# hdm0922/PathTracerDemo

Measured on AMD Instinct MI355X. Metric: Msamples/sec at 1920x1080, 1 spp ReSTIR DI; per-pixel L2 vs WebGPU ref, higher is better.
Workload: dtype f32; 1 GPU; c3_interior_32 reuse 1920x1080, 1 spp/frame (configs[2]); frame=1920x1080, band_rows_per_gpu=1080, parallelism=row-bands x1

## Files before the change

### pathtracerdemo_amd/csrc/ptx_reuse.hip

```cpp
#include "ptx_wave_common.h"

namespace ptx {

constexpr uint32_t SALT_TEMPORAL = 0x54454D50u, SALT_SPATIAL = 0x53504154u;

enum : uint32_t { JS_HDR, JS_F, JS_CUR, JS_NRM, JS_PREV, JS_RRF, JS_COUNT };
constexpr uint32_t kJobFresh = 1u << 24;
constexpr uint32_t kResReuseLayout = 0x100u;
#ifndef PTX_JOB_FRESH
#define PTX_JOB_FRESH 1
#endif

struct Job {
    uint32_t i, length, phase, seed1, idx, matref;
    uint32_t k, lab;
    bool shift, rok;
    int32_t ref;
    int32_t dom;
    f3 f;
    float prod;
    Surface cur;
    f3 prev;
    float beta, rr_p;
    f3 rr_f;
};

__device__ __forceinline__ uint32_t job_id(const ReuseArgs &A, uint32_t pix, uint32_t slot) {
    return pix * A.jpx + slot * A.jslot;
}
__device__ __forceinline__ const uint4 *res_at(const uint4 *base, int32_t idx) { return base + 8 * (ptrdiff_t)idx; }
constexpr int32_t kHistRef = 1 << 30;
__device__ __forceinline__ const uint4 *res_of(const ReuseArgs &A, int32_t ref) {
    return ref >= (kHistRef >> 1) ? A.hist + 8 * (ptrdiff_t)(ref - kHistRef) : A.cur + 8 * (ptrdiff_t)ref;
}
constexpr int32_t kDomPrev = INT32_MIN;

__device__ __forceinline__ uint32_t job_hw(const Job &s) {
    return s.i | (s.length << 8) | (s.phase << 16) | (s.lab << 18) | (s.rok ? 1u << 21 : 0u) |
           (s.shift ? 1u << 22 : 0u) | (s.k << 25);
}
__device__ __forceinline__ void job_unhw(Job &s, uint32_t hw) {
    s.i = hw & 0xffu; s.length = (hw >> 8) & 0xffu; s.phase = (hw >> 16) & 3u;
    s.lab = (hw >> 18) & 7u; s.rok = (hw >> 21) & 1u; s.shift = (hw >> 22) & 1u; s.k = (hw >> 25) & 7u;
}
__device__ __forceinline__ void job_store(const ReuseArgs &A, uint32_t jid, const Job &s) {
    const size_t n = A.njobs;
    float4 *st = A.jstate;
    if (PTX_JOB_FRESH && s.i == 1u && s.phase == 0u && s.dom != kDomPrev) {
        st[JS_HDR * n + jid] = make_float4(asf(job_hw(s) | kJobFresh), asf((uint32_t)s.dom), asf(s.idx),
                                           asf((uint32_t)s.ref));
        st[JS_F * n + jid] = make_float4(s.rr_f.x, s.rr_f.y, s.rr_f.z, s.prod);
        st[JS_RRF * n + jid] = make_float4(s.beta, s.rr_p, 0.0f, 0.0f);
        return;
    }
    st[JS_HDR * n + jid] = make_float4(asf(job_hw(s)), asf(s.seed1), asf(s.idx), asf((uint32_t)s.ref));
    st[JS_F * n + jid] = make_float4(s.f.x, s.f.y, s.f.z, s.prod);
    if (s.phase == 1u) return;
    st[JS_CUR * n + jid] = make_float4(s.cur.pos.x, s.cur.pos.y, s.cur.pos.z, asf(s.matref));
    st[JS_NRM * n + jid] = make_float4(s.cur.nrm.x, s.cur.nrm.y, s.cur.nrm.z, s.beta);
    st[JS_PREV * n + jid] = make_float4(s.prev.x, s.prev.y, s.prev.z, s.rr_p);
    st[JS_RRF * n + jid] = make_float4(s.rr_f.x, s.rr_f.y, s.rr_f.z, 0.0f);
}
__device__ __forceinline__ void job_load(const Scene &sc, const ReuseArgs &A, uint32_t jid, Job &s) {
    const size_t n = A.njobs;
    const float4 *st = A.jstate;
    const float4 hd = st[JS_HDR * n + jid], fv = st[JS_F * n + jid];
    const uint32_t hw = asu(hd.x);
    job_unhw(s, hw);
    s.idx = asu(hd.z); s.ref = (int32_t)asu(hd.w);
    s.prod = fv.w;
    const bool fresh = (hw & kJobFresh) != 0u;
    uint32_t seed1 = asu(hd.y), matref = 0u;
    int32_t dom = s.dom;
    f3 f = mk(fv.x, fv.y, fv.z), rr_f = mk(0.0f, 0.0f, 0.0f), prev = rr_f;
    float beta = 0.0f, rr_p = 0.0f;
    Surface cur{};
    if (fresh) {
        const float4 rf = st[JS_RRF * n + jid];
        dom = (int32_t)asu(hd.y);
        seed1 = res_of(A, s.ref)[0].y;
        f = mk(1.0f, 1.0f, 1.0f);
        rr_f = mk(fv.x, fv.y, fv.z);
        beta = rf.x; rr_p = rf.y;
        (void)surf_load(sc, A.surf, dom, cur, matref);
        const int32_t W = (int32_t)sc.width, q = dom >= 0 ? dom / W : -((-dom + W - 1) / W);
        prev = x0_of(sc, (uint32_t)(dom - q * W), (uint32_t)((int32_t)sc.row_begin + q));
    } else if (s.phase != 1u) {
        const float4 cu = st[JS_CUR * n + jid], nr = st[JS_NRM * n + jid];
        const float4 pv = st[JS_PREV * n + jid], rf = st[JS_RRF * n + jid];
        matref = asu(cu.w);
        cur.pos = mk(cu.x, cu.y, cu.z);
        cur.nrm = mk(nr.x, nr.y, nr.z);
        cur.mat = material_at(sc, matref);
        beta = nr.w;
        prev = mk(pv.x, pv.y, pv.z); rr_p = pv.w;
        rr_f = mk(rf.x, rf.y, rf.z);
    }
    s.seed1 = seed1; s.matref = matref; s.dom = dom;
    s.f = f; s.rr_f = rr_f; s.prev = prev;
    s.beta = beta; s.rr_p = rr_p;
    s.cur = cur;
}

__device__ __forceinline__ bool rr_step(Job &s, const Surface &X, f3 L, f3 fv, float pdf) {
    s.rr_f = s.rr_f * (fv * fabsf(dot(X.nrm, L)));
    s.rr_p *= pdf;
    const float ps = luminance(s.rr_f) / s.rr_p;
    const bool ok = ps > 0.0f;
    s.rr_p *= ps;
    if (ps > 1.0f) s.beta /= ps;
    return ok;
}

__device__ __forceinline__ void job_init(Job &s, f3 x0, const Surface &X1, uint32_t matref, int32_t ref,
                                         uint32_t length, uint32_t seed1, int32_t dom, uint32_t k, bool shift) {
    s.i = 1u; s.length = length; s.phase = 0u; s.seed1 = seed1; s.idx = 0u; s.ref = ref; s.dom = dom;
    s.k = min(k, 7u); s.lab = 0u; s.shift = shift; s.rok = false;
    s.f = mk(1.0f, 1.0f, 1.0f); s.prod = 1.0f;
    s.prev = x0;
    s.cur = X1;
    s.matref = matref;
    s.beta = 1.0f; s.rr_p = 1.0f; s.rr_f = mk(1.0f, 1.0f, 1.0f);
}
__device__ __forceinline__ bool job_begin(const Scene &sc, const ReuseArgs &A, Job &s, uint32_t x, uint32_t y,
                                          int32_t dom, int32_t ref) {
    const uint4 *rv = res_at(A.cur, ref);
    const uint4 r5 = rv[5];
    const uint32_t C = rv[7].y, length = r5.w;
    Surface X1;
    uint32_t matref;
    if (C == 0u || length < 2u || !surf_load(sc, A.surf, dom, X1, matref)) return false;
    job_init(s, x0_of(sc, x, y), X1, matref, ref, length, rv[0].y, dom, r5.x & 0xffu, false);
    return true;
}
__device__ __forceinline__ bool job_hyb(const Job &s) { return s.k >= 2u && s.k < s.length; }
__device__ __forceinline__ bool rough_under(const Surface &X, uint32_t lobe) {
    return (lobe == LOBE_LAMBERT ? 1.0f : X.mat.rough) >= RECONNECTION_ROUGHNESS;
}
__device__ __forceinline__ bool safe_edge(bool ra, bool rb, f3 a, f3 b) {
    return length(a - b) >= RECONNECTION_DISTANCE && ra && rb;
}
__device__ __forceinline__ float rc_geo(f3 prev, const Surface &Xk) {
    const f3 dv = Xk.pos - prev;
    const float d2 = dot(dv, dv);
    const float ck = fabsf(dot(Xk.nrm, dv / __builtin_sqrtf(d2)));
    return d2 / ck;
}
__device__ __forceinline__ uint4 rc_next(const uint4 *rv, uint32_t w20) {
    return (w20 & kResReuseLayout) ? rv[0] : rv[6];
}

enum : int { JK_ANY = -1, JK_L = 0, JK_C = 1, JK_B = 2 };
__device__ __forceinline__ int job_kind(uint32_t length, uint32_t k) {
    return length <= 2u ? JK_L : (k == 2u ? JK_C : JK_B);
}
template <int KIND = JK_ANY>
__device__ __forceinline__ bool job_emit(const Scene &sc, const Seg &g, const ReuseArgs &A, bool emit, Job &s,
                                         uint32_t jid, uint32_t seed0) {
    bool ray = false, vis = false, go = false;
    f3 o = mk(0.0f, 0.0f, 0.0f), d = o, Le = o;
    float remain = -1.0f;
    if (emit) {
        const uint4 *rv = res_of(A, s.ref);
        const f3 V = normalize(s.prev - s.cur.pos);
        const bool hyb = job_hyb(s);
        bool ok = true;
        if (KIND == JK_ANY ? s.i + 1u < s.length : KIND != JK_L) {
            const bool conn = KIND == JK_ANY ? s.shift && hyb && s.i + 1u == s.k : KIND == JK_C;
            const bool fixd = KIND == JK_ANY && s.shift && hyb && s.i == s.k;
            f3 dir;
            uint32_t lobe = LOBE_LAMBERT;
            if (conn || fixd) {
                const uint4 r5 = rv[5];
                const Surface Xt = get_surface(sc, gdecode(conn ? rv[4] : rc_next(rv, r5.x)));
                if (conn) {
                    const bool rk1 = rough_under(s.cur, r5.y), rk = rough_under(Xt, r5.z);
                    if (s.i >= 2u && s.lab == 0u && safe_edge(s.rok, rk1, s.prev, s.cur.pos)) s.lab = s.i;
                    if (s.lab == 0u && safe_edge(rk1, rk, s.cur.pos, Xt.pos)) s.lab = s.k;
                    ok = s.lab == s.k;
                }
                const f3 dv = Xt.pos - s.cur.pos;
                dir = dv / length(dv);
            } else {
                uint32_t seed = s.i == 1u ? seed0 : s.seed1;
                dir = sample_bsdf(seed, s.cur, V, lobe);
            }
            float pdf;
            const f3 fv = bsdf_pdf(s.cur, V, dir, pdf);
            if (!conn && !fixd && (!hyb || s.i + 2u <= s.k)) s.prod *= pdf;
            ok = rr_step(s, s.cur, dir, fv, pdf) && ok;
            if (s.shift && !conn && !fixd) {
                const bool rl = rough_under(s.cur, lobe);
                if (s.i >= 2u && s.lab == 0u && safe_edge(s.rok, rl, s.prev, s.cur.pos)) s.lab = s.i;
                s.rok = rl;
            }
            s.phase = conn ? 2u : (fixd ? 3u : 0u);
            o = s.cur.pos; d = dir;
            ray = ok && !fixd;
            go = ok;
        } else {
            const LightSample XL = load_xl(rv);
            if (s.shift && !hyb) {
                const uint32_t ll = XL.type == LIGHT_ENV ? (s.k == s.length ? rv[5].y : LOBE_GGX) : LOBE_LAMBERT;
                const bool rl = rough_under(s.cur, ll);
                if (s.i >= 2u && s.lab == 0u && safe_edge(s.rok, rl, s.prev, s.cur.pos)) s.lab = s.i;
                if (s.lab == 0u) {
                    const bool rough = s.cur.mat.rough >= RECONNECTION_ROUGHNESS;
                    const bool dirl = XL.type == LIGHT_DIRECTION || XL.type == LIGHT_ENV;
                    if ((dirl || length(s.cur.pos - XL.pos) >= RECONNECTION_DISTANCE) && rough) s.lab = s.length;
                }
                ok = s.lab == s.k;
            }
            const f3 L = direction_to_light(s.cur, XL);
            if (XL.type == LIGHT_ENV) {
                float pdf;
                const f3 fv = bsdf_pdf(s.cur, V, L, pdf);
                ok = rr_step(s, s.cur, L, fv, pdf) && ok;
            }
            s.f = s.f * (bsdf(s.cur, L, V) * fabsf(dot(s.cur.nrm, L)));
            float gl = 1.0f;
            if (XL.type == LIGHT_RECT) {
                const f3 r = XL.pos - s.cur.pos;
                const f3 Ld = normalize(r);
                gl = fabsf(dot(get_light(sc, (uint32_t)XL.id).dir, Ld)) / dot(r, r);
            }
            s.prod = hyb ? s.prod / s.beta : s.prod / (gl * s.beta);
            Le = l_emit<true>(XL, s.cur);
            s.phase = 1u;
            const float dist = length(XL.pos - s.cur.pos);
            o = s.cur.pos; d = (XL.pos - s.cur.pos) / dist; remain = dist;
            vis = true;
            ray = go = ok;
        }
        if (!go) A.jres[jid] = make_float4(0.0f, 0.0f, 0.0f, 0.0f);
    }
    const uint32_t idx = g.rbase + wave_alloc(g.l_ray, ray ? 1u : 0u);
    if (ray) {
        s.idx = idx;
        put_ray(g.rays, idx, o, d, remain, vis ? Q_VIS : Q_CLOSEST);
        if (vis) g.res_out[2u * idx] = make_float4(0.0f, Le.x, Le.y, Le.z);
    }
    return go;
}

__device__ __forceinline__ void job_finish(const Seg &g, const JobLists &JL, const ReuseArgs &A, bool live,
                                           const Job &s, uint32_t jid) {
    if (live) job_store(A, jid, s);
    const bool fold = live && A.fold_last && s.phase == 1u;
    if (fold) A.jres[jid] = make_float4(asf(s.idx), asf(g.out_sel), 0.0f, asf(kJobPending));
    job_keep(g, JL, live && !fold, live && s.phase == 1u, jid);
}

#ifndef JOB_STEP_WAVES
#define JOB_STEP_WAVES 4
#endif
__device__ __forceinline__ uint32_t job_step_segment(const Scene &sc, const WaveBufs &w, uint32_t round,
                                                     const ReuseArgs &A, uint32_t *lds) {
    const JobLists JL = job_lists(w, lds);
    const Seg g = seg_begin(w, round, lds);
    uint32_t nh;
    const uint32_t n = split_count(g, nh);
    for (uint32_t base = 0; base < n; base += WB) {
        const uint32_t q = base + threadIdx.x;
        bool emit = false;
        uint32_t jid = 0u;
        Job s;
        if (q < n) {
            jid = split_at(g, JL, q, nh);
            job_load(sc, A, jid, s);
            if (s.phase != 1u) {
                bool ok = true;
                Surface next;
                uint32_t nref = 0u;
                if (s.phase == 0u) {
                    const Hit h = get_hit(g.res_in, s.idx);
                    ok = h.valid;
                    if (ok) {
                        next = surface_at(sc, h.s, h.pos);
                        nref = mat_index(sc, h.s.inst, h.s.mat);
                    }
                } else {
                    const uint4 *rv = res_of(A, s.ref);
                    const Compact cc = gdecode(s.phase == 2u ? rv[4] : rc_next(rv, rv[5].x));
                    next = get_surface(sc, cc);
                    nref = mat_index(sc, cc.inst, cc.mat);
                    if (s.phase == 2u) {
                        const Hit h = get_hit(g.res_in, s.idx);
                        ok = !(h.valid && h.t < length(next.pos - s.cur.pos) * 0.999f);
                    }
                }
                if (!ok) {
                    A.jres[jid] = make_float4(0.0f, 0.0f, 0.0f, 0.0f);
                } else {
                    const f3 V = normalize(s.prev - s.cur.pos);
                    const f3 L = normalize(next.pos - s.cur.pos);
                    s.f = s.f * (bsdf(s.cur, L, V) * fabsf(dot(s.cur.nrm, L)));
                    if (s.phase == 2u || (!s.shift && job_hyb(s) && s.i + 1u == s.k))
                        s.prod = s.prod * rc_geo(s.cur.pos, next);
                    s.prev = s.cur.pos;
                    s.cur = next;
                    s.matref = nref;
                    s.i += 1u;
                    emit = true;
                }
            } else {
                const float4 a = g.res_in[2u * s.idx];
                s.f = s.f * (mk(a.y, a.z, a.w) * a.x);
                const float qv = s.prod;
                const bool valid = qv > 0.0f && qv <= 3.402823466e38f;
                A.jres[jid] = valid ? make_float4(s.f.x, s.f.y, s.f.z, qv) : make_float4(0.0f, 0.0f, 0.0f, 0.0f);
            }
        }
        const bool live = job_emit(sc, g, A, emit, s, jid, 0u);
        job_finish(g, JL, A, live, s, jid);
    }
    job_seg_end(w, g, JL);
    return *g.l_ray;
}
__global__ __launch_bounds__(WB) __attribute__((amdgpu_waves_per_eu(JOB_STEP_WAVES, 8)))
void wjob_step(Scene sc, WaveBufs w, uint32_t round, ReuseArgs A) {
    PTX_WAVE_TIMER(sc, KID_JOB_STEP | (w.seg_base ? 0x80u : 0u));
    __shared__ uint32_t lds[3];
    (void)job_step_segment(sc, w, round, A, lds);
}

__device__ __forceinline__ uint32_t reuse_seed(const Scene &sc, uint32_t x, uint32_t y, uint32_t salt) {
    return pcg(pcg(x * 1973u + y * 9277u + sc.U[U_FRAME] * 26699u) ^ salt);
}
__device__ __forceinline__ bool wrs_update(float &w_sum, float wt, uint32_t &seed) {
    w_sum += wt;
    return rnd(seed) < wt / w_sum;
}
struct SelF { bool known; f3 f; };
__device__ __forceinline__ SelF job_f(float4 r) { return SelF{r.w > 0.0f, mk(r.x, r.y, r.z)}; }
__device__ __forceinline__ float4 job_result(const ReuseArgs &A, const WaveBufs &w, float4 r, uint32_t jid) {
    if (asu(r.w) != kJobPending || asu(r.x) >= A.ray_cap || asu(r.y) >= w.nres) return r;
    const float4 a = w.res[asu(r.y)][2u * asu(r.x)], fv = A.jstate[JS_F * (size_t)A.njobs + jid];
    const f3 f = mk(fv.x, fv.y, fv.z) * (mk(a.y, a.z, a.w) * a.x);
    const float qv = fv.w;
    const bool valid = qv > 0.0f && qv <= 3.402823466e38f;
    return valid ? make_float4(f.x, f.y, f.z, qv) : make_float4(0.0f, 0.0f, 0.0f, 0.0f);
}
__device__ __forceinline__ float4 job_at(const ReuseArgs &A, const WaveBufs &w, uint32_t pix, uint32_t slot) {
    const uint32_t jid = job_id(A, pix, slot);
    return job_result(A, w, A.jres[jid], jid);
}
__device__ __forceinline__ SelF stored_f(const uint4 *r) {
    const uint4 r6 = r[6], r7 = r[7];
    return SelF{r7.w == 1u, mk(asf(r6.z), asf(r6.w), asf(r7.z))};
}
__device__ __forceinline__ void write_reused(uint4 *out, const uint4 *src, float p_sel, float q_sel, SelF fs,
                                             float w_sum, uint32_t C) {
    uint4 a0 = src[0], a5 = src[5];
    const uint4 a1 = src[1], a2 = src[2], a3 = src[3], a4 = src[4];
    if (fs.known && !(a5.x & kResReuseLayout)) {
        const uint32_t k = a5.x & 0xffu;
        if (k >= 2u && k + 1u < a5.w) a0 = src[6];
        a5.x |= kResReuseLayout;
    }
    out[0] = a0; out[1] = a1; out[2] = a2; out[3] = a3; out[4] = a4; out[5] = a5;
    out[6] = make_uint4(asu(p_sel), asu(q_sel), fs.known ? asu(fs.f.x) : 0u, fs.known ? asu(fs.f.y) : 0u);
    out[7] = make_uint4(asu(p_sel > 0.0f ? w_sum / p_sel : 0.0f), C, fs.known ? asu(fs.f.z) : 0u, fs.known ? 1u : 0u);
}

constexpr uint32_t kNbrEscape = 0xFFFFFFFFu;
__device__ __forceinline__ uint4 nbr_pack(bool valid, uint4 r5, uint4 r6, uint4 r7) {
    uint32_t w = 0u;
    const uint32_t k = r5.x & 0xffu;
    if (valid)
        w = (r5.w > 0xfu || k > 0xfu || r7.y > 0x7ffffeu) ? kNbrEscape : (1u << 31) | (r5.w << 27) | (k << 23) | r7.y;
    return make_uint4(r6.x, r6.y, r7.x, w);
}

__device__ __forceinline__ bool temporal_from_init(const Scene &sc, const WaveBufs &w, const ReuseArgs &A, Job &s,
                                                   uint32_t pix, uint32_t jid) {
    const uint4 *rv = res_at(A.cur, s.ref);
    const bool hyb = job_hyb(s);
    while (s.i + 1u < s.length) {
        f3 V = normalize(s.prev - s.cur.pos);
        uint32_t seed = s.i == 1u ? rv[0].x : s.seed1, lobe;
        const f3 dir = sample_bsdf(seed, s.cur, V, lobe);
        float pdf;
        const f3 fv = bsdf_pdf(s.cur, V, dir, pdf);
        if (!hyb || s.i + 2u <= s.k) s.prod *= pdf;
        if (!rr_step(s, s.cur, dir, fv, pdf)) {
            A.jres[jid] = make_float4(0.0f, 0.0f, 0.0f, 0.0f);
            return false;
        }
        const float4 c = w.state[(s.i == 1u ? kStateCs2 : kStateCs3) * w.npix + pix];
        const Surface next = get_surface(sc, gdecode(make_uint4(asu(c.x), asu(c.y), asu(c.z), asu(c.w))));
        V = normalize(s.prev - s.cur.pos);
        const f3 L = normalize(next.pos - s.cur.pos);
        s.f = s.f * (bsdf(s.cur, L, V) * fabsf(dot(s.cur.nrm, L)));
        if (hyb && s.i + 1u == s.k) s.prod = s.prod * rc_geo(s.cur.pos, next);
        s.prev = s.cur.pos;
        s.cur = next;
        s.i += 1u;
    }
    const float T = w.state[kStateTsel * w.npix + pix].x;
    if (T < 0.0f) return true;
    const LightSample XL = load_xl(rv);
    const f3 V = normalize(s.prev - s.cur.pos);
    const f3 L = direction_to_light(s.cur, XL);
    s.f = s.f * (bsdf(s.cur, L, V) * fabsf(dot(s.cur.nrm, L)));
    float gl = 1.0f;
    if (XL.type == LIGHT_RECT) {
        const f3 r = XL.pos - s.cur.pos;
        const f3 Ld = normalize(r);
        gl = fabsf(dot(get_light(sc, (uint32_t)XL.id).dir, Ld)) / dot(r, r);
    }
    s.prod = hyb ? s.prod / s.beta : s.prod / (gl * s.beta);
    const f3 Le = l_emit<true>(XL, s.cur);
    s.f = s.f * (Le * T);
    const float qv = s.prod;
    const bool valid = qv > 0.0f && qv <= 3.402823466e38f;
    A.jres[jid] = valid ? make_float4(s.f.x, s.f.y, s.f.z, qv) : make_float4(0.0f, 0.0f, 0.0f, 0.0f);
    return false;
}

__global__ __launch_bounds__(WB) __attribute__((amdgpu_waves_per_eu(2, 8)))
void wtemporal_start(Scene sc, WaveBufs w, ReuseArgs A) {
    PTX_WAVE_TIMER(sc, KID_TEMP_START | (w.seg_base ? 0x80u : 0u));
    __shared__ uint32_t lds[3];
    const JobLists JL = job_lists(w, lds);
    const Seg g = seg_begin(w, 0u, lds);
    const uint32_t np = padded_pixels(sc);
    for (uint32_t k = 0; k < w.seg_px; k += WB) {
        const uint32_t q = seg_pixel(w, g.j, k);
        uint32_t x, y, pix = 0u;
        bool active = false;
        Job s;
        if (q < np && tile_xy(sc, q, x, y)) {
            pix = (y - sc.row_begin) * sc.width + x;
            active = job_begin(sc, A, s, x, y, (int32_t)pix, (int32_t)pix);
            if (active && A.use_init) active = temporal_from_init(sc, w, A, s, pix, pix);
        }
        const bool live = job_emit(sc, g, A, active, s, pix, active ? A.cur[8u * (size_t)pix].x : 0u);
        job_finish(g, JL, A, live, s, pix);
    }
    job_seg_end(w, g, JL);
}

__global__ __launch_bounds__(WB) void wtemporal_combine(Scene sc, WaveBufs w, ReuseArgs A) {
    PTX_WAVE_TIMER(sc, KID_TEMP_COMBINE | (w.seg_base ? 0x80u : 0u));
    const uint32_t j = w.seg_base + blockIdx.x, np = padded_pixels(sc);
    for (uint32_t k = 0; k < w.seg_px; k += WB) {
        const uint32_t q = seg_pixel(w, j, k);
        uint32_t x, y;
        if (q >= np || !tile_xy(sc, q, x, y)) continue;
        const uint32_t pix = (y - sc.row_begin) * sc.width + x;
        if (!gdecode(A.gbuf[pix]).valid) {
            A.nbr_out[pix] = make_uint4(0u, 0u, 0u, 0u);
            continue;
        }
        uint4 *rv = A.cur + 8u * (size_t)pix;
        const uint4 *hv = A.hist + 8u * (size_t)pix;
        uint32_t seed = reuse_seed(sc, x, y, SALT_TEMPORAL);
        const uint4 r5 = rv[5], r7 = rv[7];
        const float4 er = (r7.y != 0u && r5.w >= 2u) ? job_result(A, w, A.jres[pix], pix) : make_float4(0.0f, 0.0f, 0.0f, 0.0f);
        const float2 ec = make_float2(er.w > 0.0f ? luminance(mk(er.x, er.y, er.z)) : 0.0f, er.w);
        const bool canon_ok = ec.y > 0.0f && ec.x > 0.0f;
        const uint4 h5 = hv[5], h6 = hv[6], h7 = hv[7];
        const uint32_t Cp = A.hist_valid ? min(h7.y, A.cap) : 0u;
        const float cp = (float)Cp, tot = 1.0f + cp;
// ... 632 lines not shown
```

### pathtracerdemo_amd/csrc/ptx_shading.h

```cpp
#pragma once

#include "ptx_device.h"

namespace ptx {

struct Material { f3 albedo; float metal, rough, trans, ior; };
struct Surface { f3 pos, nrm; Material mat; };

__device__ __forceinline__ uint32_t mat_index(const Scene &sc, uint32_t inst, uint32_t sub) {
    return sc.insts[inst].sub_base + sub;
}
__device__ __forceinline__ Material material_at(const Scene &sc, uint32_t flat) {
    const float4 a = sc.mats[2u * flat], b = sc.mats[2u * flat + 1u];
    Material m;
    m.albedo = mk(a.x, a.y, a.z);
    m.metal = a.w;
    m.rough = b.x;
    m.trans = b.y;
    m.ior = b.z;
    return m;
}
__device__ __forceinline__ float get_transmission(const Scene &sc, uint32_t inst, uint32_t mid) {
    return sc.mats[2u * mat_index(sc, inst, mid) + 1u].y;
}
__device__ __forceinline__ float subs_transmission(const SubRoot *subs, const Inst *insts, uint32_t inst, uint32_t mid) {
    return asf(subs[insts[inst].sub_base + mid].pad);
}

__device__ __forceinline__ Surface get_surface(const Scene &sc, Compact x) {
    const Inst &I = sc.insts[x.inst];
    Surface s;
    s.mat = material_at(sc, I.sub_base + x.mat);
    const TriVerts tv = tri_verts(sc, I.tri_base + x.prim);
    f3 p0 = inst_point(I, I.m, tv.p[0]);
    f3 n0 = inst_point_t(I, I.minv, tv.n[0]);
    f3 p1 = inst_point(I, I.m, tv.p[1]);
    f3 n1 = inst_point_t(I, I.minv, tv.n[1]);
    f3 p2 = inst_point(I, I.m, tv.p[2]);
    f3 n2 = inst_point_t(I, I.minv, tv.n[2]);
    float U = x.bu, V = x.bv, W = 1.0f - U - V;
    s.nrm = normalize((n0 * U + n1 * V) + n2 * W);
    s.pos = (p0 * U + p1 * V) + p2 * W;
    return s;
}
__device__ __forceinline__ Surface surface_at(const Scene &sc, const Compact &x, f3 pos) {
    const Inst &I = sc.insts[x.inst];
    Surface s;
    s.mat = material_at(sc, I.sub_base + x.mat);
    const TriVerts tv = tri_verts(sc, I.tri_base + x.prim);
    f3 n0 = inst_point_t(I, I.minv, tv.n[0]);
    f3 n1 = inst_point_t(I, I.minv, tv.n[1]);
    f3 n2 = inst_point_t(I, I.minv, tv.n[2]);
    float U = x.bu, V = x.bv, W = 1.0f - U - V;
    s.nrm = normalize((n0 * U + n1 * V) + n2 * W);
    s.pos = pos;
    return s;
}
__device__ __forceinline__ f3 get_surface_pos(const Scene &sc, Compact x) {
    const Inst &I = sc.insts[x.inst];
    const TriVerts tv = tri_verts(sc, I.tri_base + x.prim);
    f3 p0 = inst_point(I, I.m, tv.p[0]);
    f3 p1 = inst_point(I, I.m, tv.p[1]);
    f3 p2 = inst_point(I, I.m, tv.p[2]);
    float U = x.bu, V = x.bv, W = 1.0f - U - V;
    return (p0 * U + p1 * V) + p2 * W;
}

struct Light { f3 pos, dir, color, U, V; uint32_t type; float intensity, area; };
struct LightSample { f3 dir; uint32_t type; f3 pos; int32_t id; f3 Le; float pdf; };

__device__ __forceinline__ Light get_light(const Scene &sc, uint32_t id) {
    const uint32_t *p = sc.S + sc.U[U_OFF_LIGHT] + STRIDE_LIGHT * id;
    Light l;
    l.pos = mk(asf(p[0]), asf(p[1]), asf(p[2]));
    l.dir = mk(asf(p[3]), asf(p[4]), asf(p[5]));
    l.color = mk(asf(p[6]), asf(p[7]), asf(p[8]));
    l.U = mk(asf(p[9]), asf(p[10]), asf(p[11]));
    l.V = mk(asf(p[12]), asf(p[13]), asf(p[14]));
    l.type = p[15];
    l.intensity = asf(p[16]);
    l.area = asf(p[17]);
    return l;
}
__device__ __forceinline__ float light_cdf(const Scene &sc, uint32_t i) { return asf(sc.S[sc.U[U_OFF_CDF] + i]); }

__device__ __forceinline__ float ggx_d(float NdotH, float R) {
    float a = R * R, a2 = a * a;
    float X = NdotH * NdotH * (a2 - 1.0f) + 1.0f;
    float denom = PI_F * X * X;
    return a2 / fmaxf(denom, EPS_F);
}
__device__ __forceinline__ float geom_shadow(float NdotV, float NdotL, float R) {
    float r = R + 1.0f;
    float K = r * r / 8.0f;
    return 1.0f / ((NdotV * (1.0f - K) + K) * (NdotL * (1.0f - K) + K));
}
__device__ __forceinline__ float pow5(float x) {
    float x2 = x * x;
    return (x2 * x2) * x;
}
__device__ __forceinline__ void fsincos(float x, float &s, float &c) {
    int j = (int)(x * 1.27323954473516f);
    float y = (float)j;
    if (j & 1) {
        j += 1;
        y += 1.0f;
    }
    j &= 7;
    float z = ((x - y * 0.78515625f) - y * 2.4187564849853515625e-4f) - y * 3.77489497744594108e-8f;
    float zz = z * z;
    float ps = ((-1.9515295891e-4f * zz + 8.3321608736e-3f) * zz - 1.6666654611e-1f) * zz * z + z;
    float pc = ((2.443315711809948e-5f * zz - 1.388731625493765e-3f) * zz + 4.166664568298827e-2f) * zz * zz -
               0.5f * zz + 1.0f;
    const bool swap = (j & 2) != 0;
    const float sv = swap ? pc : ps, cv = swap ? ps : pc;
    s = (j == 4 || j == 6) ? -sv : sv;
    c = (j == 2 || j == 4) ? -cv : cv;
}
__device__ __forceinline__ f3 fresnel(float d, f3 F0) {
    float p = pow5(1.0f - saturate(d));
    return mk(F0.x + (1.0f - F0.x) * p, F0.y + (1.0f - F0.y) * p, F0.z + (1.0f - F0.z) * p);
}
__device__ __forceinline__ f3 brdf(const Surface &X, f3 V, f3 L) {
    f3 N = X.nrm;
    f3 H = normalize(L + V);
    float NdotV = fmaxf(dot(N, V), 0.0f), NdotL = fmaxf(dot(N, L), 0.0f);
    float NdotH = fmaxf(dot(N, H), 0.0f), VdotH = fmaxf(dot(V, H), 0.0f);
    f3 base = X.mat.albedo;
    float metal = X.mat.metal, R = X.mat.rough;
    f3 F0 = mix3(mk(0.04f, 0.04f, 0.04f), base, metal);
    float D = ggx_d(NdotH, R);
    float G0 = geom_shadow(NdotV, NdotL, R);
    f3 F = fresnel(VdotH, F0);
    f3 kD = mk(1.0f - F.x, 1.0f - F.y, 1.0f - F.z) * (1.0f - metal);
    f3 diffuse = (kD / PI_F) * base;
    f3 spec = ((F * D) * G0) * 0.25f;
    return diffuse + spec;
}
__device__ __forceinline__ f3 btdf(const Surface &X, f3 V, f3 L) {
    float R = X.mat.rough;
    bool same = dot(V, X.nrm) > 0.0f;
    float n_in = same ? X.mat.ior : 1.0f;
    float n_out = same ? 1.0f : X.mat.ior;
    f3 hv = L * n_in + V * n_out;
    float H_norm = length(hv);
    f3 N = same ? X.nrm : -X.nrm;
    f3 H = normalize(hv);
    float NdotL = fabsf(dot(N, L)), NdotV = fabsf(dot(N, V)), NdotH = fabsf(dot(N, H));
    float LdotH = fabsf(dot(L, H)), VdotH = fabsf(dot(V, H));
    float G0 = geom_shadow(NdotL, NdotV, R);
    float D = ggx_d(NdotH, R);
    float nr = (n_out - n_in) / (n_out + n_in);
    f3 F = fresnel(LdotH, mk(nr * nr, nr * nr, nr * nr));
    f3 num = mk(1.0f - F.x, 1.0f - F.y, 1.0f - F.z) * (n_out * n_out);
    num = ((((num * LdotH) * VdotH) * G0) * D) * X.mat.albedo;
    return num / fmaxf(H_norm * H_norm, EPS_F);
}
__device__ __forceinline__ f3 bsdf(const Surface &X, f3 V, f3 L) {
    float T = X.mat.trans;
    if (dot(L, X.nrm) * dot(V, X.nrm) > 0.0f) return brdf(X, V, L) * (1.0f - T);
    return btdf(X, V, L) * T;
}

struct Tbn { f3 T, B, N; };
__device__ __forceinline__ Tbn tbn(f3 N) {
    bool same = fabsf(dot(N, mk(0.0f, 1.0f, 0.0f))) > 0.9999f;
    f3 cv = same ? mk(1.0f, 0.0f, 0.0f) : mk(0.0f, 1.0f, 0.0f);
    Tbn m;
    m.T = normalize(cross(cv, N));
    m.B = cross(N, m.T);
    m.N = N;
    return m;
}
__device__ __forceinline__ f3 tbn_mul(const Tbn &m, f3 v) { return (m.T * v.x + m.B * v.y) + m.N * v.z; }
__device__ __forceinline__ f3 reflect3(f3 I, f3 N) { return I - N * (2.0f * dot(N, I)); }
__device__ __forceinline__ f3 refract3(f3 I, f3 N, float eta) {
    float d = dot(N, I);
    float k = 1.0f - eta * eta * (1.0f - d * d);
    if (k < 0.0f) return mk(0.0f, 0.0f, 0.0f);
    return I * eta - N * (eta * d + __builtin_sqrtf(k));
}
__device__ __forceinline__ f3 sample_cosine(uint32_t &seed) {
    float r1 = rnd(seed), r2 = rnd(seed);
    float R = __builtin_sqrtf(r1);
    float phi = 2.0f * PI_F * r2, sp, cp;
    fsincos(phi, sp, cp);
    return mk(R * cp, R * sp, __builtin_sqrtf(1.0f - r1));
}
__device__ __forceinline__ f3 sample_ggx(uint32_t &seed, float R) {
    float r1 = rnd(seed), r2 = rnd(seed);
    float a = R * R;
    float phi = 2.0f * PI_F * r1;
    float ct = __builtin_sqrtf((1.0f - r2) / (1.0f + (a * a - 1.0f) * r2));
    float st = __builtin_sqrtf(1.0f - ct * ct), sp, cp;
    fsincos(phi, sp, cp);
    return normalize(mk(st * cp, st * sp, ct));
}
__device__ __forceinline__ f3 sample_bsdf(uint32_t &seed, const Surface &X, f3 V, uint32_t &lobe) {
    bool transparent = rnd(seed) < X.mat.trans;
    if (transparent) {
        bool same = dot(V, X.nrm) > 0.0f;
        float n_in = same ? 1.0f : X.mat.ior;
        float n_out = same ? X.mat.ior : 1.0f;
        f3 N = same ? X.nrm : -X.nrm;
        float ratio = n_in / n_out;
        float r = (1.0f - ratio) / (1.0f + ratio);
        float R2 = ratio * ratio;
        float cos_t = fabsf(dot(V, N));
// ... 183 lines not shown
```

### pathtracerdemo_amd/csrc/ptx_wave_common.h

```cpp
#pragma once
#include "ptx_launch.h"
#include "ptx_shading.h"

namespace ptx {

constexpr uint32_t WB = kBlock;
#ifndef LOGIC_WAVES
#define LOGIC_WAVES 4
#endif
enum : uint32_t { Q_CLOSEST = 0u, Q_VIS = 1u, Q_OCC = 2u };

__device__ __forceinline__ uint32_t wave_scan(uint32_t v, uint32_t &total) { return wave_excl_sum(v, total); }
__device__ __forceinline__ uint32_t wave_alloc(uint32_t *lds_ctr, uint32_t n) {
    uint32_t total;
    const uint32_t excl = wave_scan(n, total);
    uint32_t base = 0u;
    if (__lane_id() == 0u && total) base = atomicAdd(lds_ctr, total);
    base = (uint32_t)__builtin_amdgcn_readfirstlane((int)base);
    return base + excl;
}

struct Seg {
    uint32_t j, round;
    uint32_t pj;
    uint32_t rbase;
    float4 *rays, *res_out;
    const float4 *res_in;
    uint32_t out_sel;
    uint32_t *act_out;
    const uint32_t *act_in;
    uint32_t n_in;
    uint32_t *l_ray, *l_act;
};
__device__ __forceinline__ uint32_t res_sel(const WaveBufs &w, uint32_t round) {
    return w.nres == 3u ? round % 3u : round & 1u;
}
__device__ __forceinline__ float4 *res_buf(const WaveBufs &w, uint32_t round) { return w.res[res_sel(w, round)]; }
__device__ __forceinline__ Seg seg_begin(const WaveBufs &w, uint32_t round, uint32_t *lds) {
    Seg g;
    g.j = w.seg_base + blockIdx.x;
    g.pj = w.seg_phys + g.j;
    g.round = round;
    g.rbase = g.pj * w.ray_stride;
    g.rays = w.rays;
    g.res_out = res_buf(w, round);
    g.res_in = round ? res_buf(w, round - 1u) : w.res[1];
    g.out_sel = res_sel(w, round);
    g.act_out = w.act[round & 1u] + (size_t)g.pj * w.act_stride;
    g.act_in = w.act[(round + 1u) & 1u] + (size_t)g.pj * w.act_stride;
    g.n_in = round ? w.cnt[(2u * (round - 1u)) * w.cnt_stride + g.pj] : 0u;
    g.l_ray = lds;
    g.l_act = lds + 1;
    if (threadIdx.x == 0) { lds[0] = 0u; lds[1] = 0u; }
    if (w.dyn && blockIdx.x == 0 && threadIdx.x < kDynHeads) w.dyn[round * kDynRoundWords + threadIdx.x * kDynStride] = 0u;
    __syncthreads();
    return g;
}
__device__ __forceinline__ void seg_end(const WaveBufs &w, const Seg &g) {
    __syncthreads();
    if (threadIdx.x == 0) {
        w.cnt[(2u * g.round) * w.cnt_stride + g.pj] = *g.l_act;
        w.cnt[(2u * g.round + 1u) * w.cnt_stride + g.pj] = *g.l_ray;
    }
}
__device__ __forceinline__ uint32_t set_tile(const WaveBufs &w, uint32_t v) {
    return v < w.ntile0 ? w.tile0 + v : v - w.ntile0 < w.ntile1 ? w.tile1 + (v - w.ntile0) : 0x3ffffffu;
}
__device__ __forceinline__ uint32_t seg_pixel(const WaveBufs &w, uint32_t j, uint32_t k) {
    const uint32_t s = (k + threadIdx.x) >> 6;
    const uint32_t cl = w.cluster;
    const uint32_t t = set_tile(w, ((s / cl) * w.nseg + j) * cl + s % cl);
    return t * 64u + (threadIdx.x & 63u);
}
__device__ __forceinline__ void seg_keep(const Seg &g, bool keep, uint32_t pix) {
    const uint32_t slot = wave_alloc(g.l_act, keep ? 1u : 0u);
    if (keep) g.act_out[slot] = pix;
}

struct JobLists { uint32_t *l_light; uint32_t stride; };
__device__ __forceinline__ JobLists job_lists(const WaveBufs &w, uint32_t *lds) {
    if (threadIdx.x == 0) lds[2] = 0u;
    return JobLists{lds + 2, w.act_stride};
}
__device__ __forceinline__ void job_keep(const Seg &g, const JobLists &L, bool keep, bool light, uint32_t jid) {
    const uint32_t sh = wave_alloc(g.l_act, keep && !light ? 1u : 0u);
    const uint32_t sl = wave_alloc(L.l_light, keep && light ? 1u : 0u);
    if (keep) g.act_out[light ? L.stride - 1u - sl : sh] = jid;
}
__device__ __forceinline__ void job_seg_end(const WaveBufs &w, const Seg &g, const JobLists &L) {
    __syncthreads();
    if (threadIdx.x == 0) {
        w.cnt[(2u * g.round) * w.cnt_stride + g.pj] = *g.l_act | (*L.l_light << 16);
        w.cnt[(2u * g.round + 1u) * w.cnt_stride + g.pj] = *g.l_ray;
    }
}

__device__ __forceinline__ uint32_t split_count(const Seg &g, uint32_t &nh) {
    nh = g.n_in & 0xffffu;
    return nh + (g.n_in >> 16);
}
__device__ __forceinline__ uint32_t split_at(const Seg &g, const JobLists &L, uint32_t q, uint32_t nh) {
    return g.act_in[q < nh ? q : L.stride - 1u - (q - nh)];
}

__device__ __forceinline__ void put_ray(float4 *rays, uint32_t idx, f3 o, f3 d, float remain, uint32_t kind) {
    rays[2u * idx] = make_float4(o.x, o.y, o.z, remain);
    rays[2u * idx + 1u] = make_float4(d.x, d.y, d.z, asf(kind));
}
__device__ __forceinline__ Hit get_hit(const float4 *res, uint32_t idx) {
    const float4 a = res[2u * idx], b = res[2u * idx + 1u];
    const uint32_t enc = asu(a.y);
    Hit h;
    h.valid = (enc >> 31) != 0u;
    h.t = a.x;
    h.s = Compact{enc >> 31, (enc >> 16) & 0x7fffu, enc & 0xffffu, asu(a.z), a.w, b.x};
    h.pos = mk(b.y, b.z, b.w);
    return h;
}
__device__ __forceinline__ f3 x0_of(const Scene &sc, uint32_t x, uint32_t y) {
    const float *vpinv = reinterpret_cast<const float *>(sc.U + U_VPINV);
    float u = ((float)x + 0.5f) / (float)sc.U[U_W];
    float v = ((float)y + 0.5f) / (float)sc.U[U_H];
    return xform_point(vpinv, mk(2.0f * u - 1.0f, 2.0f * v - 1.0f, 0.0f));
}
__device__ __forceinline__ Compact gdecode(uint4 g) {
    return Compact{(g.x & 0x80000000u) ? 1u : 0u, (g.x & 0x7fff0000u) >> 16, g.x & 0xffffu, g.y, asf(g.z), asf(g.w)};
}
__device__ __forceinline__ uint4 gencode(const Compact &s) {
    return make_uint4((s.valid << 31) | (s.inst << 16) | s.mat, s.prim, asu(s.bu), asu(s.bv));
}
__device__ __forceinline__ void mix_color(const Scene &sc, float4 *accum, uint32_t i, f3 c) {
    float t = 1.0f / (float)(sc.U[U_FRAME] + 1u);
    float4 a = accum[i];
    accum[i] = make_float4(mixf(a.x, c.x, t), mixf(a.y, c.y, t), mixf(a.z, c.z, t), 1.0f);
}
__device__ __forceinline__ bool tile_xy(const Scene &sc, uint32_t p, uint32_t &x, uint32_t &y) {
    const uint32_t tiles_x = (sc.width + 7u) / 8u, t = p >> 6, l = p & 63u;
    x = (t % tiles_x) * 8u + (l & 7u);
    y = sc.row_begin + (t / tiles_x) * 8u + (l >> 3);
    return x < sc.width && y < sc.row_end;
}
__device__ __forceinline__ uint32_t padded_pixels(const Scene &sc) {
    return ((sc.width + 7u) / 8u) * ((sc.row_end - sc.row_begin + 7u) / 8u) * 64u;
}

constexpr uint32_t kNoSurface = 0xFFFFFFFFu;
__device__ __forceinline__ void surf_store(uint4 *surf, ptrdiff_t i, const Surface &X, uint32_t matref) {
    surf[2 * i] = make_uint4(asu(X.pos.x), asu(X.pos.y), asu(X.pos.z), matref);
    surf[2 * i + 1] = make_uint4(asu(X.nrm.x), asu(X.nrm.y), asu(X.nrm.z), 0u);
}
__device__ __forceinline__ void surf_store_none(uint4 *surf, ptrdiff_t i) {
    surf[2 * i] = make_uint4(0u, 0u, 0u, kNoSurface);
}
__device__ __forceinline__ bool surf_load(const Scene &sc, const uint4 *surf, ptrdiff_t i, Surface &X,
                                          uint32_t &matref) {
    const uint4 a = surf[2 * i];
    if (a.w == kNoSurface) return false;
    const uint4 b = surf[2 * i + 1];
    X.pos = mk(asf(a.x), asf(a.y), asf(a.z));
    X.nrm = mk(asf(b.x), asf(b.y), asf(b.z));
    X.mat = material_at(sc, a.w);
    matref = a.w;
    return true;
}
__device__ __forceinline__ void surf_from_gbuf(const Scene &sc, uint4 *surf, ptrdiff_t i, uint4 g) {
    const Compact x1 = gdecode(g);
    if (!x1.valid) surf_store_none(surf, i);
    else surf_store(surf, i, get_surface(sc, x1), mat_index(sc, x1.inst, x1.mat));
}

__device__ __forceinline__ LightSample load_xl(const uint4 *res) {
    const uint4 r1 = res[1], r2 = res[2], r3 = res[3];
    LightSample XL;
    XL.dir = mk(asf(r1.x), asf(r1.y), asf(r1.z));
    XL.type = r1.w;
    XL.pos = mk(asf(r2.x), asf(r2.y), asf(r2.z));
    XL.id = (int32_t)r2.w;
    XL.Le = mk(asf(r3.x), asf(r3.y), asf(r3.z));
    XL.pdf = asf(r3.w);
    return XL;
}
}
```

Measured before the change: 564.0 Msamples/s.

## Hoist and flatten job-step global loads to issue them before dependent shading

Restructures the job-step loop so every global load is issued early and predicated on phase flags rather than sitting in nested branches: job header, job body, hit records, reservoir entries, material and instance data. The goal is more memory-level parallelism and less divergence-serialized latency per wave. Fresh jobs now read the surface buffer straight through the body loader instead of calling surf_load, and a new surface_of takes precomputed instance refs. The cost is higher register pressure from keeping more values live, plus some loads that may now be wasted for lanes that won't use them.

```diff
diff --git a/pathtracerdemo_amd/csrc/ptx_reuse.hip b/pathtracerdemo_amd/csrc/ptx_reuse.hip
--- a/pathtracerdemo_amd/csrc/ptx_reuse.hip
+++ b/pathtracerdemo_amd/csrc/ptx_reuse.hip
@@ -61,40 +61,56 @@
     st[JS_PREV * n + jid] = make_float4(s.prev.x, s.prev.y, s.prev.z, s.rr_p);
     st[JS_RRF * n + jid] = make_float4(s.rr_f.x, s.rr_f.y, s.rr_f.z, 0.0f);
 }
-__device__ __forceinline__ void job_load(const Scene &sc, const ReuseArgs &A, uint32_t jid, Job &s) {
+struct JobBody { float4 fv, rrf, cur, nrm, prev; uint32_t seed1; };
+__device__ __forceinline__ float4 job_head(const ReuseArgs &A, uint32_t jid) {
+    return A.jstate[JS_HDR * (size_t)A.njobs + jid];
+}
+__device__ __forceinline__ JobBody job_body(const ReuseArgs &A, uint32_t jid, float4 hd, bool has, bool heavy,
+                                            bool fresh) {
     const size_t n = A.njobs;
     const float4 *st = A.jstate;
-    const float4 hd = st[JS_HDR * n + jid], fv = st[JS_F * n + jid];
-    const uint32_t hw = asu(hd.x);
-    job_unhw(s, hw);
+    const float4 z = make_float4(0.0f, 0.0f, 0.0f, 0.0f);
+    JobBody B{z, z, z, z, z, 0u};
+    if (has) B.fv = st[JS_F * n + jid];
+    if (heavy) {
+        const float4 *sf = reinterpret_cast<const float4 *>(A.surf) + 2 * (ptrdiff_t)(fresh ? (int32_t)asu(hd.y) : 0);
+        B.rrf = st[JS_RRF * n + jid];
+        B.cur = *(fresh ? sf : st + (JS_CUR * n + jid));
+        B.nrm = *(fresh ? sf + 1 : st + (JS_NRM * n + jid));
+    }
+    if (heavy && !fresh) B.prev = st[JS_PREV * n + jid];
+    if (fresh) B.seed1 = res_of(A, (int32_t)asu(hd.w))[0].y;
+    return B;
+}
+__device__ __forceinline__ void job_unpack(const Scene &sc, float4 hd, const JobBody &B, const Material &mat,
+                                           bool heavy, bool fresh, Job &s) {
+    const float4 fv = B.fv;
+    job_unhw(s, asu(hd.x));
     s.idx = asu(hd.z); s.ref = (int32_t)asu(hd.w);
     s.prod = fv.w;
-    const bool fresh = (hw & kJobFresh) != 0u;
     uint32_t seed1 = asu(hd.y), matref = 0u;
-    int32_t dom = s.dom;
+    int32_t dom = 0;
     f3 f = mk(fv.x, fv.y, fv.z), rr_f = mk(0.0f, 0.0f, 0.0f), prev = rr_f;
     float beta = 0.0f, rr_p = 0.0f;
     Surface cur{};
     if (fresh) {
-        const float4 rf = st[JS_RRF * n + jid];
         dom = (int32_t)asu(hd.y);
-        seed1 = res_of(A, s.ref)[0].y;
+        seed1 = B.seed1;
         f = mk(1.0f, 1.0f, 1.0f);
         rr_f = mk(fv.x, fv.y, fv.z);
-        beta = rf.x; rr_p = rf.y;
-        (void)surf_load(sc, A.surf, dom, cur, matref);
+        beta = B.rrf.x; rr_p = B.rrf.y;
         const int32_t W = (int32_t)sc.width, q = dom >= 0 ? dom / W : -((-dom + W - 1) / W);
         prev = x0_of(sc, (uint32_t)(dom - q * W), (uint32_t)((int32_t)sc.row_begin + q));
-    } else if (s.phase != 1u) {
-        const float4 cu = st[JS_CUR * n + jid], nr = st[JS_NRM * n + jid];
-        const float4 pv = st[JS_PREV * n + jid], rf = st[JS_RRF * n + jid];
-        matref = asu(cu.w);
-        cur.pos = mk(cu.x, cu.y, cu.z);
-        cur.nrm = mk(nr.x, nr.y, nr.z);
-        cur.mat = material_at(sc, matref);
-        beta = nr.w;
-        prev = mk(pv.x, pv.y, pv.z); rr_p = pv.w;
-        rr_f = mk(rf.x, rf.y, rf.z);
+    } else if (heavy) {
+        beta = B.nrm.w;
+        prev = mk(B.prev.x, B.prev.y, B.prev.z); rr_p = B.prev.w;
+        rr_f = mk(B.rrf.x, B.rrf.y, B.rrf.z);
+    }
+    if (heavy) {
+        matref = asu(B.cur.w);
+        cur.pos = mk(B.cur.x, B.cur.y, B.cur.z);
+        cur.nrm = mk(B.nrm.x, B.nrm.y, B.nrm.z);
+        cur.mat = mat;
     }
     s.seed1 = seed1; s.matref = matref; s.dom = dom;
     s.f = f; s.rr_f = rr_f; s.prev = prev;
@@ -260,56 +276,62 @@
     const Seg g = seg_begin(w, round, lds);
     uint32_t nh;
     const uint32_t n = split_count(g, nh);
+    const float4 z4 = make_float4(0.0f, 0.0f, 0.0f, 0.0f);
+    const uint4 zu = make_uint4(0u, 0u, 0u, 0u);
     for (uint32_t base = 0; base < n; base += WB) {
         const uint32_t q = base + threadIdx.x;
+        const bool has = q < n;
+        const uint32_t jid = has ? split_at(g, JL, q, nh) : 0u;
+        const float4 hd = has ? job_head(A, jid) : z4;
+        Job s;
+        job_unhw(s, asu(hd.x));
+        const uint32_t idx = asu(hd.z);
+        const bool heavy = has && s.phase != 1u, light = has && s.phase == 1u;
+        const bool fresh = has && (asu(hd.x) & kJobFresh) != 0u;
+        const uint4 *rv = res_of(A, (int32_t)asu(hd.w));
+        const JobBody B = job_body(A, jid, hd, has, heavy, fresh);
+        float4 ha = z4, hb = z4;
+        if (has && s.phase != 3u) ha = g.res_in[2u * idx];
+        if (has && s.phase == 0u) hb = g.res_in[2u * idx + 1u];
+        uint4 ca = zu;
+        uint32_t w20 = 0u;
+        if (heavy && s.phase == 2u) ca = rv[4];
+        if (heavy && s.phase == 3u) w20 = rv[5].x;
+        if (heavy && s.phase == 3u) ca = rc_next(rv, w20);
+        Material cmat{};
+        if (heavy) cmat = material_at(sc, asu(B.cur.w));
+        const Hit h = hit_of(ha, hb);
+        const Compact cc = s.phase == 0u ? h.s : gdecode(ca);
+        bool ok = heavy && (s.phase != 0u || h.valid);
+        InstRef ir{0u, 0u, 0u};
+        if (ok) ir = inst_ref(sc, cc.inst);
+        Surface next{};
+        if (ok) next = surface_of(sc, cc, ir, s.phase == 0u, h.pos);
+        const uint32_t nref = ir.sub_base + cc.mat;
+        job_unpack(sc, hd, B, cmat, heavy, fresh, s);
         bool emit = false;
-        uint32_t jid = 0u;
-        Job s;
-        if (q < n) {
-            jid = split_at(g, JL, q, nh);
-            job_load(sc, A, jid, s);
-            if (s.phase != 1u) {
-                bool ok = true;
-                Surface next;
-                uint32_t nref = 0u;
-                if (s.phase == 0u) {
-                    const Hit h = get_hit(g.res_in, s.idx);
-                    ok = h.valid;
-                    if (ok) {
-                        next = surface_at(sc, h.s, h.pos);
-                        nref = mat_index(sc, h.s.inst, h.s.mat);
-                    }
-                } else {
-                    const uint4 *rv = res_of(A, s.ref);
-                    const Compact cc = gdecode(s.phase == 2u ? rv[4] : rc_next(rv, rv[5].x));
-                    next = get_surface(sc, cc);
-                    nref = mat_index(sc, cc.inst, cc.mat);
-                    if (s.phase == 2u) {
-                        const Hit h = get_hit(g.res_in, s.idx);
-                        ok = !(h.valid && h.t < length(next.pos - s.cur.pos) * 0.999f);
-                    }
-                }
-                if (!ok) {
-                    A.jres[jid] = make_float4(0.0f, 0.0f, 0.0f, 0.0f);
-                } else {
-                    const f3 V = normalize(s.prev - s.cur.pos);
-                    const f3 L = normalize(next.pos - s.cur.pos);
-                    s.f = s.f * (bsdf(s.cur, L, V) * fabsf(dot(s.cur.nrm, L)));
-                    if (s.phase == 2u || (!s.shift && job_hyb(s) && s.i + 1u == s.k))
-                        s.prod = s.prod * rc_geo(s.cur.pos, next);
-                    s.prev = s.cur.pos;
-                    s.cur = next;
-                    s.matref = nref;
-                    s.i += 1u;
-                    emit = true;
-                }
+        if (heavy) {
+            if (ok && s.phase == 2u)
+                ok = !(h.valid && h.t < length(next.pos - s.cur.pos) * 0.999f);
+            if (!ok) {
+                A.jres[jid] = make_float4(0.0f, 0.0f, 0.0f, 0.0f);
             } else {
-                const float4 a = g.res_in[2u * s.idx];
-                s.f = s.f * (mk(a.y, a.z, a.w) * a.x);
-                const float qv = s.prod;
-                const bool valid = qv > 0.0f && qv <= 3.402823466e38f;
-                A.jres[jid] = valid ? make_float4(s.f.x, s.f.y, s.f.z, qv) : make_float4(0.0f, 0.0f, 0.0f, 0.0f);
-            }
+                const f3 V = normalize(s.prev - s.cur.pos);
+                const f3 L = normalize(next.pos - s.cur.pos);
+                s.f = s.f * (bsdf(s.cur, L, V) * fabsf(dot(s.cur.nrm, L)));
+                if (s.phase == 2u || (!s.shift && job_hyb(s) && s.i + 1u == s.k))
+                    s.prod = s.prod * rc_geo(s.cur.pos, next);
+                s.prev = s.cur.pos;
+                s.cur = next;
+                s.matref = nref;
+                s.i += 1u;
+                emit = true;
+            }
+        } else if (light) {
+            s.f = s.f * (mk(ha.y, ha.z, ha.w) * ha.x);
+            const float qv = s.prod;
+            const bool valid = qv > 0.0f && qv <= 3.402823466e38f;
+            A.jres[jid] = valid ? make_float4(s.f.x, s.f.y, s.f.z, qv) : make_float4(0.0f, 0.0f, 0.0f, 0.0f);
         }
         const bool live = job_emit(sc, g, A, emit, s, jid, 0u);
         job_finish(g, JL, A, live, s, jid);
diff --git a/pathtracerdemo_amd/csrc/ptx_shading.h b/pathtracerdemo_amd/csrc/ptx_shading.h
--- a/pathtracerdemo_amd/csrc/ptx_shading.h
+++ b/pathtracerdemo_amd/csrc/ptx_shading.h
@@ -54,6 +54,37 @@
     float U = x.bu, V = x.bv, W = 1.0f - U - V;
     s.nrm = normalize((n0 * U + n1 * V) + n2 * W);
     s.pos = pos;
+    return s;
+}
+struct InstRef { uint32_t mesh, sub_base, tri_base; };
+__device__ __forceinline__ InstRef inst_ref(const Scene &sc, uint32_t inst) {
+    const Inst &I = sc.insts[inst];
+    return InstRef{I.mesh, I.sub_base, I.tri_base};
+}
+__device__ __forceinline__ Surface surface_of(const Scene &sc, const Compact &x, InstRef r, bool has_pos, f3 pos) {
+    const Inst &I = sc.insts[x.inst];
+    Surface s;
+    s.mat = material_at(sc, r.sub_base + x.mat);
+    const TriVerts tv = tri_verts(sc, r.tri_base + x.prim);
+    const bool ident = (r.mesh & kInstIdentity) != 0u;
+    float U = x.bu, V = x.bv, W = 1.0f - U - V;
+    s.pos = pos;
+    if (!has_pos) {
+        f3 p[3];
+#pragma unroll
+        for (int v = 0; v < 3; ++v) {
+            const f3 q = tv.p[v];
+            p[v] = (ident && finite3(q)) ? f3{q.x + 0.0f, q.y + 0.0f, q.z + 0.0f} : xform_point(I.m, q);
+        }
+        s.pos = (p[0] * U + p[1] * V) + p[2] * W;
+    }
+    f3 n[3];
+#pragma unroll
+    for (int v = 0; v < 3; ++v) {
+        const f3 q = tv.n[v];
+        n[v] = (ident && finite3(q)) ? f3{q.x + 0.0f, q.y + 0.0f, q.z + 0.0f} : xform_point_t(I.minv, q);
+    }
+    s.nrm = normalize((n[0] * U + n[1] * V) + n[2] * W);
     return s;
 }
 __device__ __forceinline__ f3 get_surface_pos(const Scene &sc, Compact x) {
diff --git a/pathtracerdemo_amd/csrc/ptx_wave_common.h b/pathtracerdemo_amd/csrc/ptx_wave_common.h
--- a/pathtracerdemo_amd/csrc/ptx_wave_common.h
+++ b/pathtracerdemo_amd/csrc/ptx_wave_common.h
@@ -107,8 +107,7 @@
     rays[2u * idx] = make_float4(o.x, o.y, o.z, remain);
     rays[2u * idx + 1u] = make_float4(d.x, d.y, d.z, asf(kind));
 }
-__device__ __forceinline__ Hit get_hit(const float4 *res, uint32_t idx) {
-    const float4 a = res[2u * idx], b = res[2u * idx + 1u];
+__device__ __forceinline__ Hit hit_of(float4 a, float4 b) {
     const uint32_t enc = asu(a.y);
     Hit h;
     h.valid = (enc >> 31) != 0u;
@@ -116,6 +115,9 @@
     h.s = Compact{enc >> 31, (enc >> 16) & 0x7fffu, enc & 0xffffu, asu(a.z), a.w, b.x};
     h.pos = mk(b.y, b.z, b.w);
     return h;
+}
+__device__ __forceinline__ Hit get_hit(const float4 *res, uint32_t idx) {
+    return hit_of(res[2u * idx], res[2u * idx + 1u]);
 }
 __device__ __forceinline__ f3 x0_of(const Scene &sc, uint32_t x, uint32_t y) {
     const float *vpinv = reinterpret_cast<const float *>(sc.U + U_VPINV);
```

New measurement: 564.9 Msamples/s (median of 3 runs). No clear change (+0.2%).
